# batra-mlp-lab/visdial

Hardware: AMD Instinct MI355X
Metric: QA-rounds/sec training mn-att-ques-im-hist+disc (batch 20x10x100) (higher is better)
Workload: dtype f32 operands and results; the option recurrence multiplies the EXACT 3-way bf16 split of both operands (9 bf16 MFMA products per fp32 product, f32 accumulate: fp32-grade, errors at the f32 MFMA's own level) -- its two step kernels and its weight-gradient contraction; f32 MFMA (v_mfma_f32_32x32x2_f32

## Files before the change

### visdial_amd/csrc/rt_core.h

```cpp
#pragma once
#include <math.h>
#include <stdarg.h>
#include <stdlib.h>
#include <string.h>

#include <algorithm>
#include <map>
#include <memory>
#include <numeric>
#include <random>
#include <string>
#include <vector>

#include "../../include/visdial_hip.h"
#include "common.h"
#include "paths.h"

int vd_lstm2_forward_p(const vd_lstm2_fwd_t* st, int nstacks, int H, int flags, hipStream_t stream);
int vd_lstm2_backward_p(const vd_lstm2_bwd_t* st, int nstacks, int H, int flags, hipStream_t stream);

int vd_img_drop_gather(const float* pre, const uint8_t* mask1, float* xdrop, int N, int R, int S2, int H, float scale, hipStream_t stream);
int vd_img_common_forward_p(const float* pre, const uint8_t* mask1, const float* xdrop, const float* Wc, const float* bc, const float* qc,
                            const uint8_t* mask2, float* iqc, int N, int R, int S2, int H, int Kc, float scale, int flags, hipStream_t stream);
int vd_img_tr_backward_p(const float* dz, const float* Wc, const float* p, const float* datt, const uint8_t* mask1, float* dpre, int N, int R,
// ... 123 lines not shown
  void flush() {
    index.reset(index.T);
    ++stamp;
  }
};
static constexpr long VD_OPTION_CACHE_DEFAULT_ROWS = 262144;
static constexpr long VD_OPTION_CACHE_FIRST_ROWS = 16384;

struct Encoder;
struct Decoder;

}

struct vd_model {
  vd_model_params p;
  int flags = 0;
  std::string enc_name, dec_name;
  std::vector<vdrt::Tensor> spec;
  std::map<std::string, int> index;
  long numel = 0;
  float *W = nullptr, *G = nullptr, *M = nullptr, *V = nullptr;
  std::map<std::string, vdrt::DevBuf> ws;
  std::map<std::string, vdrt::DevBuf> ext_masks;
  hipStream_t s_main = nullptr, s_enc = nullptr, s_img = nullptr, s_hist = nullptr, s_tab = nullptr, s_copy = nullptr;
  hipStream_t s_wg = nullptr;
  bool wg_active = false, wg_used = false;
  std::vector<hipEvent_t> ev_pool;
  size_t ev_next = 0;
  hipEvent_t ev_enc_grads = nullptr;
  hipEvent_t ev_updated = nullptr;
  bool updated_recorded = false;
  bool enc_grads_recorded = false;
  hipEvent_t ev_loss = nullptr, ev_prof[6] = {nullptr, nullptr, nullptr, nullptr, nullptr, nullptr};
  bool training = true, streams = true, prof_valid = false;
  long step = 0;
  int adam_t = 0;
  double lr = 1e-3;
  vdrt::BatchSlot slot[2];
  int cur = -1, uploaded = -1;
  float* loss_host = nullptr;
  long loss_cap = 0, loss_n = 0;
  bool loss_is_sum = false;
  std::unique_ptr<vdrt::Encoder> enc;
  std::unique_ptr<vdrt::Decoder> dec;
  float* scores = nullptr;
  float* gen_enc_out = nullptr;
  int gen_seq_len = 0;
// ... 42 lines not shown
}

inline void add_lstm(vd_model* m, const std::string& name, long D, long H) {
  m->spec.push_back(Tensor{name + ".W", 0, D + H, 4 * H, 1});
  m->spec.push_back(Tensor{name + ".b", 0, 1, 4 * H, 2});
}
inline void add_linear(vd_model* m, const std::string& name, long in, long out) {
  m->spec.push_back(Tensor{name + ".W", 0, out, in, 3});
  m->spec.push_back(Tensor{name + ".b", 0, 1, out, 4});
}
inline std::string hop_sfx(int i) { return i == 0 ? std::string() : std::to_string(i + 1); }

inline float* Wp(vd_model* m, const std::string& n) { return m->W + m->spec[m->index.at(n)].off; }
inline float* Gp(vd_model* m, const std::string& n) { return m->G + m->spec[m->index.at(n)].off; }

inline int fork_stream(vd_model* m, hipStream_t from, hipStream_t side) {
  if (side == from) return VD_OK;
  hipEvent_t e = m->ev_pool[m->ev_next++ % m->ev_pool.size()];
  VD_HIP(hipEventRecord(e, from));
  VD_HIP(hipStreamWaitEvent(side, e, 0));
  return VD_OK;
}
inline int join_stream(vd_model* m, hipStream_t side, hipStream_t to) { return fork_stream(m, side, to); }
inline hipStream_t side_stream(vd_model* m, hipStream_t wanted, hipStream_t cur) { return m->streams ? wanted : cur; }
inline int wg_fork(vd_model* m, hipStream_t cur, hipStream_t* out) {
  *out = cur;
  if (!m->wg_active || !m->s_wg) return VD_OK;
  VD_TRY(fork_stream(m, cur, m->s_wg));
  m->wg_used = true;
  *out = m->s_wg;
  return VD_OK;
}

inline int drop_mask(vd_model* m, const std::string& site, size_t numel, float p, hipStream_t s, uint8_t** out) {
  *out = nullptr;
  if (!m->training || p <= 0.f) return VD_OK;
  auto it = m->ext_masks.find(site);
  if (it != m->ext_masks.end()) {
    VD_CHECK_ARG(it->second.bytes >= numel, "dropout mask '%s' holds %zu bytes, the batch needs %zu", site.c_str(),
                 it->second.bytes, numel);
    *out = static_cast<uint8_t*>(it->second.p);
    return VD_OK;
  }
  if (!m->ext_masks.empty()) {
    vd_set_error("external dropout masks are set but none for site '%s'", site.c_str());
    return VD_ERR_STATE;
  }
// ... 300 lines not shown
```

### visdial_amd/csrc/rt_decoders.h

```cpp
#pragma once
#include "rt_encoders.h"

namespace vdrt {

int option_cache_resolve(vd_model* m, BatchSlot& sl, const int32_t* options, long NO, int To, hipStream_t s);

struct Decoder {
  virtual ~Decoder() {}
  virtual void declare(vd_model* m) = 0;
  virtual int forward_backward(vd_model* m, BatchSlot& b, bool only_forward) = 0;
  virtual int retrieve(vd_model* m, BatchSlot& b) = 0;
  virtual int retrieve_lhood(vd_model*, BatchSlot&) {
    vd_set_error("vd_model_retrieve_lhood: the live-row log-likelihood head scores candidates of decoder 'gen'; this model's decoder is 'disc'");
    return VD_ERR_ARG;
  }
  virtual int gen_begin(vd_model*, const int32_t*, int) { return no_gen(); }
  virtual int gen_step(vd_model*, const int32_t*, float*) { return no_gen(); }
  virtual int gen_select(vd_model*, const int32_t*, int) { return no_gen(); }
  virtual int gen_beam_search(vd_model*, int, int, int, int, int32_t*, double*) { return no_gen(); }
  virtual int gen_sample(vd_model*, int, int, int, double, const double*, int32_t*, double*) { return no_gen(); }
  static int no_gen() {
    vd_set_error("sampling / beam search only for the generative decoder (model.lua:436-438)");
    return VD_ERR_STATE;
  }
// ... 15 lines not shown

#ifdef VD_PROBE_PHASES
inline hipEvent_t* probe_events() {
  static hipEvent_t e[6];
  static bool made = false;
  if (!made) { for (auto& x : e) (void)hipEventCreate(&x); made = true; }
  return e;
}
#define VD_PROBE_REC(i, stream) (void)hipEventRecord(probe_events()[i], stream)
#else
#define VD_PROBE_REC(i, stream)
#endif
struct Disc : Decoder {
  void declare(vd_model* m) override { add_lstm(m, "opt", m->p.embedSize, m->p.rnnHiddenSize); }
  int forward_backward(vd_model* m, BatchSlot& b, bool only_forward) override {
    VD_CHECK_ARG(b.opt.present, "decoder 'disc' needs batch.options");
    VD_CHECK_ARG(only_forward || b.has_gt, "training decoder 'disc' needs batch.answer_ind");
    if (b.cached) return forward_cached(m, b, only_forward);
    const int N = b.q.N, O = m->p.numOptions, NOfull = N * O, NO = b.opt.N, To = b.opt.T;
    const bool dedup = b.opt_uid != nullptr;
    VD_CHECK_ARG(dedup ? NO <= NOfull : NO == NOfull, "decoder 'disc': %d option rows for %d x %d candidates", NO, N, O);
    const long H = m->p.rnnHiddenSize, E = m->p.embedSize, V = m->p.vocabSize;
    hipStream_t s = m->s_main;
    hipStream_t se = side_stream(m, m->s_enc, s);
    hipStream_t st = side_stream(m, m->s_tab, s);
    float *table, *gates, *h, *c, *scores, *loss_rows;
    VD_TRY(ws_get(m, "opt.table", (size_t)(V + 1) * 4 * H, &table));
    VD_TRY(ws_get(m, "opt.gates", (size_t)To * NO * 4 * H, &gates));
    VD_TRY(ws_get(m, "opt.h", (size_t)To * NO * H, &h));
    VD_TRY(ws_get(m, "opt.c", (size_t)To * NO * H, &c));
    VD_TRY(ws_get(m, "opt.scores", (size_t)N * O, &scores));
    VD_TRY(ws_get(m, "crit.loss_rows", (size_t)N, &loss_rows));
    float* Wopt = Wp(m, "opt.W");
    const int flags = m->flags;
    VD_TRY(fork_stream(m, s, se));
    float* enc_out = nullptr;
    VD_TRY(vd_gemm_nn(Wp(m, "embed"), E, Wopt, 4 * H, Wp(m, "opt.b"), table, 4 * H, (int)V + 1, (int)(4 * H), (int)E, 0, s));
    const bool c16 = (flags & VD_FLAG_BF16) && vd_lstm_c16_fits(NO, (int)H);
    vd_bf16_bits *gates16 = reinterpret_cast<vd_bf16_bits*>(gates), *h16 = reinterpret_cast<vd_bf16_bits*>(h), *table16 = nullptr;
    float* h_last = nullptr;
    if (c16) {
      float* t16;
      VD_TRY(ws_get(m, "opt.table16", (size_t)(V + 1) * 2 * H, &t16));
      VD_TRY(ws_get(m, "opt.h_last", (size_t)NO * H, &h_last));
      table16 = reinterpret_cast<vd_bf16_bits*>(t16);
      VD_TRY(vd_f32_to_bf16(table, table16, (V + 1) * 4 * H, s));
    }
    VD_HIP(hipEventRecord(m->ev_prof[0], s));
    {
      VdRange r("disc: option LSTM forward");
      if (c16) VD_TRY(vd_lstm_forward_c16(table16, 4 * H, b.opt.tok, Wopt + E * 4 * H, gates16, h16, h_last, c, To, NO, (int)H, s));
      else VD_TRY(vd_lstm_forward(table, 0, 4 * H, b.opt.tok, nullptr, Wopt + E * 4 * H, nullptr, nullptr, gates, h, c, To, NO, (int)H, flags, s));
    }
    VD_HIP(hipEventRecord(m->ev_prof[1], s));
    {
      VdRange r("encoder forward");
      VD_TRY(m->enc->forward(m, se, b, &enc_out));
      VD_PROBE_REC(0, se);
    }
    VD_TRY(join_stream(m, se, s));
    const float* optH = c16 ? h_last : h + (long)(To - 1) * NO * H;
    float *d_optH = nullptr, *d_enc = nullptr, *d_optH_full = nullptr;
    if (dedup) {
      float* full;
      VD_TRY(ws_get(m, "opt.h_full", (size_t)NOfull * H, &full));
      VD_TRY(vd_embed_gather(optH, b.opt_uid, nullptr, full, NOfull, (int)H, 1.f, s));
      optH = full;
    }
    if (!only_forward) {
      VD_TRY(ws_get(m, "crit.d_optH", (size_t)NO * H, &d_optH));
      VD_TRY(ws_get(m, "crit.d_enc", (size_t)N * H, &d_enc));
      if (dedup) VD_TRY(ws_get(m, "crit.d_optH_full", (size_t)NOfull * H, &d_optH_full));
    }
    VD_TRY(vd_score_ce(optH, enc_out, b.gt, scores, loss_rows, dedup ? d_optH_full : d_optH, d_enc, N, O, (int)H, 1.0f / N, s));
    if (dedup && !only_forward) {
      VD_TRY(vd_memset(d_optH, 0, (long)NO * H * 4, s));
      VD_TRY(vd_embed_scatter_acc(d_optH, b.opt_uid, nullptr, d_optH_full, NOfull, (int)H, 1.f, s));
    }
    VD_TRY(stage_loss(m, loss_rows, N, false, s));
    m->scores = scores;
    m->prof_valid = !only_forward;
    if (only_forward) return VD_OK;
    VD_TRY(fork_stream(m, s, se));
    float *dc, *dtab;
    int32_t* perm = b.opt_sort_perm;
    VD_TRY(ws_get(m, "opt.dc", (size_t)NO * H, &dc));
    VD_TRY(ws_get(m, "opt.dtable", (size_t)(V + 1) * 4 * H, &dtab));
    VD_CHECK_ARG(perm, "decoder 'disc': the batch slot carries no option-token sort");
    VD_TRY(fork_stream(m, s, st));
    VD_TRY(vd_memset(dtab, 0, (V + 1) * 4 * H * 4, st));
    VD_HIP(hipEventRecord(m->ev_prof[2], s));
    m->wg_active = m->streams && m->s_wg && (flags & VD_FLAG_BF16) != 0;
    m->wg_used = false;
    auto enc_bwd = [&]() -> int {
      VdRange r("encoder backward");
      VD_TRY(m->enc->backward(m, se, b, d_enc));
      VD_PROBE_REC(1, se);
      if (m->wg_used) VD_PROBE_REC(2, m->s_wg);
      if (m->wg_used) {
        VD_TRY(fork_stream(m, se, m->s_wg));
        VD_HIP(hipEventRecord(m->ev_enc_grads, m->s_wg));
      } else {
        VD_HIP(hipEventRecord(m->ev_enc_grads, se));
      }
      m->enc_grads_recorded = true;
      return VD_OK;
    };
    {
      VdRange r("disc: option LSTM backward");
      if (c16) VD_TRY(vd_lstm_backward_c16(Wopt + E * 4 * H, gates16, c, d_optH, dc, To, NO, (int)H, s));
      else VD_TRY(vd_lstm_backward(Wopt + E * 4 * H, gates, c, nullptr, nullptr, d_optH, nullptr, dc, nullptr, nullptr, nullptr, To, NO, (int)H, flags, s));
    }
    VD_HIP(hipEventRecord(m->ev_prof[3], s));
    VD_TRY(enc_bwd());
    VdRange rwg("disc: table gradient + dWh");
    VD_TRY(fork_stream(m, s, st));
    if (c16) VD_TRY(vd_segment_rowsum_acc_bf16(gates16, 4 * H, b.opt.tok, perm, (long)To * NO, (int)(4 * H), dtab, 4 * H, st));
    else VD_TRY(vd_segment_rowsum_acc(gates, 4 * H, b.opt.tok, perm, (long)To * NO, (int)(4 * H), dtab, 4 * H, st));
    VD_TRY(vd_colsum_acc(dtab, 4 * H, (int)V + 1, (int)(4 * H), Gp(m, "opt.b"), st));
    VD_TRY(vd_gemm_tn_acc(Wp(m, "embed"), E, dtab, 4 * H, Gp(m, "opt.W"), 4 * H, (int)E, (int)(4 * H), (int)V + 1, 0, st));
    VD_HIP(hipEventRecord(m->ev_prof[4], s));
    if (To > 1 && c16)
      VD_TRY(vd_gemm_tn_acc_bf16(h16, gates16 + (long)NO * 4 * H, Gp(m, "opt.W") + E * 4 * H, 4 * H, (int)H, (int)(4 * H), (To - 1) * NO, s));
    else if (To > 1)
      VD_TRY(vd_gemm_tn_acc(h, H, gates + (long)NO * 4 * H, 4 * H, Gp(m, "opt.W") + E * 4 * H, 4 * H, (int)H, (int)(4 * H), (To - 1) * NO,
                            flags & (VD_FLAG_BF16 | VD_FLAG_SPLIT9), s));
    VD_HIP(hipEventRecord(m->ev_prof[5], s));
    VD_TRY(vd_gemm_nt(dtab, 4 * H, Wopt, 4 * H, nullptr, Gp(m, "embed"), E, (int)V + 1, (int)E, (int)(4 * H), VD_ACT_NONE, 2, st));
    VD_PROBE_REC(3, st);
    VD_TRY(join_stream(m, se, s));
    if (m->wg_used) VD_TRY(join_stream(m, m->s_wg, s));
    m->wg_active = m->wg_used = false;
    VD_TRY(join_stream(m, st, s));
    VD_PROBE_REC(4, s);
    return VD_OK;
  }
  int retrieve(vd_model* m, BatchSlot& b) override { return forward_backward(m, b, true); }

  int forward_cached(vd_model* m, BatchSlot& b, bool only_forward) {
    if (!only_forward || m->training) {
      vd_set_error("decoder 'disc': this batch was uploaded for cached evaluation (VD_OPTION_CACHE with training off) and carries only the "
                   "candidate rows the cache did not hold; upload it again after vd_model_set_training(1) for a training step");
      return VD_ERR_STATE;
    }
    OptionCache& oc = m->ocache;
    const int N = b.q.N, O = m->p.numOptions, NOfull = N * O, To = b.opt.T;
    const long H = m->p.rnnHiddenSize, E = m->p.embedSize, V = m->p.vocabSize;
    hipStream_t s = m->s_main;
    hipStream_t se = side_stream(m, m->s_enc, s);
    if (b.cache_stamp != oc.stamp) {
      VD_HIP(hipEventSynchronize(b.ready));
      VD_TRY(option_cache_resolve(m, b, b.opt_host.data(), NOfull, To, s));
      VD_HIP(hipStreamSynchronize(s));
    }
    const int U = b.opt.N;
    const long count = oc.index.size();
    VD_CHECK_ARG(b.opt_total == NOfull && (long)b.miss_keys.size() == (long)U * To && count <= oc.capacity,
                 "decoder 'disc': inconsistent cached batch (%d candidates, %d misses)", b.opt_total, U);
    if (oc.table_rows < count + U) {
      const long want = std::min(std::max(2 * oc.table_rows, VD_OPTION_CACHE_FIRST_ROWS), oc.capacity);
      const long rows = std::max(want, count + U);
      float* nt = nullptr;
      VD_HIP(hipMalloc((void**)&nt, (size_t)rows * H * sizeof(float)));
      if (oc.table) {
        if (count > 0) VD_HIP(hipMemcpyAsync(nt, oc.table, (size_t)count * H * sizeof(float), hipMemcpyDeviceToDevice, s));
        VD_HIP(hipStreamSynchronize(s));
        VD_HIP(hipFree(oc.table));
      }
      oc.table = nt;
      oc.table_rows = rows;
    }
    float *scores, *loss_rows, *full;
    VD_TRY(ws_get(m, "opt.scores", (size_t)N * O, &scores));
    VD_TRY(ws_get(m, "crit.loss_rows", (size_t)N, &loss_rows));
    VD_TRY(ws_get(m, "opt.h_full", (size_t)NOfull * H, &full));
    VD_TRY(fork_stream(m, s, se));
    if (U > 0) {
      VdRange r("disc: option LSTM forward (state only, cache misses)");
      float *table, *h, *c;
      VD_TRY(ws_get(m, "opt.table", (size_t)(V + 1) * 4 * H, &table));
      VD_TRY(ws_get(m, "opt.h2", (size_t)2 * U * H, &h));
      VD_TRY(ws_get(m, "opt.c2", (size_t)2 * U * H, &c));
      float* Wopt = Wp(m, "opt.W");
      VD_TRY(vd_gemm_nn(Wp(m, "embed"), E, Wopt, 4 * H, Wp(m, "opt.b"), table, 4 * H, (int)V + 1, (int)(4 * H), (int)E, 0, s));
      VD_TRY(vd_lstm_forward(table, 0, 4 * H, b.opt.tok, nullptr, Wopt + E * 4 * H, nullptr, nullptr, nullptr, h, c, To, U, (int)H,
                             m->flags | VD_FLAG_STATE_ONLY, s));
      VD_HIP(hipMemcpyAsync(oc.table + count * H, h + (long)((To - 1) & 1) * U * H, (size_t)U * H * sizeof(float), hipMemcpyDeviceToDevice, s));
      const long fit = std::min<long>(U, oc.capacity - count);
      for (long i = 0; i < fit; ++i) oc.index.add(b.miss_keys.data() + (size_t)i * To);
    }
    ++oc.stamp;
    float* enc_out = nullptr;
    {
      VdRange r("encoder forward");
      VD_TRY(m->enc->forward(m, se, b, &enc_out));
    }
    VD_TRY(join_stream(m, se, s));
    VD_TRY(vd_embed_gather(oc.table, b.opt_uid, nullptr, full, NOfull, (int)H, 1.f, s));
    VD_TRY(vd_score_ce(full, enc_out, b.gt, scores, loss_rows, nullptr, nullptr, N, O, (int)H, 1.0f / N, s));
    VD_TRY(stage_loss(m, loss_rows, N, false, s));
    m->scores = scores;
    m->prof_valid = false;
    return VD_OK;
  }
};

struct Gen;
int Gen_begin(Gen* g, vd_model* m, const int32_t* rounds, int n);
int Gen_step(Gen* g, vd_model* m, const int32_t* tokens, float* host_logp);
int Gen_select(Gen* g, vd_model* m, const int32_t* src, int n_keep);
int Gen_beam_search(Gen* g, vd_model* m, int k, int L, int start, int end, int32_t* host_tokens, double* host_scores);
int Gen_sample(Gen* g, vd_model* m, int L, int start, int end, double T, const double* host_u, int32_t* host_tokens,
               double* host_loglik);

struct Gen : Decoder {
  int gen_begin(vd_model* m, const int32_t* r, int n) override { return Gen_begin(this, m, r, n); }
  int gen_step(vd_model* m, const int32_t* t, float* lp) override { return Gen_step(this, m, t, lp); }
  int gen_select(vd_model* m, const int32_t* src, int k) override { return Gen_select(this, m, src, k); }
  int gen_beam_search(vd_model* m, int k, int L, int st, int en, int32_t* t, double* sc) override {
    return Gen_beam_search(this, m, k, L, st, en, t, sc);
// ... 453 lines not shown
```

### visdial_amd/csrc/rt_encoders.h

```cpp
#pragma once
#include "rt_core.h"

namespace vdrt {

struct Encoder {
  virtual ~Encoder() {}
  virtual void declare(vd_model* m) = 0;
  virtual int forward(vd_model* m, hipStream_t s, BatchSlot& b, float** out) = 0;
  virtual int backward(vd_model* m, hipStream_t s, BatchSlot& b, const float* grad_out) = 0;
  virtual std::vector<SeqLSTM>* rnnLayers() { return nullptr; }
  virtual int seqLen(const BatchSlot& b) const { return b.q.T; }
};

inline int tick_flags(const vd_model* m) { return m->flags & VD_FLAG_BF16; }

inline int causal_mask(vd_model* m, int B, int R, uint8_t** out) {
  const std::string key = "causal." + std::to_string(B);
  DevBuf& d = m->ws[key];
  const size_t n = (size_t)B * R * R;
  if (!d.p) {
    std::vector<uint8_t> host(n);
    for (int r = 0; r < B * R; ++r)
      for (int j = 0; j < R; ++j) host[(size_t)r * R + j] = j > (r % R) ? 1 : 0;
    VD_HIP(hipMalloc(&d.p, n + 16));
// ... 224 lines not shown
  std::vector<float*> iqc, patt;
  float sc = 1.f;
  float* xdrop = nullptr;
  int iflags = 0;
  static void declare(vd_model* m) {
    const long H = m->p.rnnHiddenSize, C = m->p.imgFeatureSize, K = m->p.commonEmbeddingSize;
    add_linear(m, "img_proj", C, H);
    for (int i = 0; i < std::max(1, m->p.numAttentionLayers); ++i) {
      add_linear(m, "img_common" + hop_sfx(i), H, K);
      add_linear(m, "ques_common" + hop_sfx(i), H, K);
      add_linear(m, "att" + hop_sfx(i), K, 1);
    }
    add_linear(m, "out", H, H);
  }
  void init(vd_model* m) {
    H = m->p.rnnHiddenSize; C = m->p.imgFeatureSize; K = m->p.commonEmbeddingSize;
    S2 = m->p.imgSpatialSize * m->p.imgSpatialSize; R = m->p.maxQuesCount; L = std::max(1, m->p.numAttentionLayers);
    img_proj.init("img_proj", C, H); out.init("out", H, H);
    ques_common.resize(L);
    for (int i = 0; i < L; ++i) ques_common[i].init("ques_common" + hop_sfx(i), H, K);
  }
  int prefetch(vd_model* m, hipStream_t s, BatchSlot& b, int N_) {
    N = N_;
    hipStream_t si = side_stream(m, m->s_img, s);
    VD_TRY(fork_stream(m, s, si));
    VD_TRY(img_proj.forward(m, si, b.img, (long)b.B * S2, true, &pre));
    VD_TRY(drop_mask(m, "img_tr", (size_t)N * S2 * H, 0.5f, si, &m1));
    m2.assign(L, nullptr);
    for (int i = 0; i < L; ++i) VD_TRY(drop_mask(m, "iqc" + hop_sfx(i), (size_t)N * S2 * K, 0.5f, si, &m2[i]));
    sc = m1 ? 2.f : 1.f;
    iflags = (m->flags & VD_FLAG_SPLIT9) && vd_img_split_ok((long)N * S2, (int)H, (int)K) ? VD_FLAG_SPLIT9 : 0;
    xdrop = nullptr;
    if (iflags) {
      VD_TRY(ws_get(m, "att.xdrop", (size_t)N * S2 * H, &xdrop));
      VD_TRY(vd_img_drop_gather(pre, m1, xdrop, N, R, S2, (int)H, sc, si));
    }
    return VD_OK;
  }
  int forward(vd_model* m, hipStream_t s, const float* u0, float** y) {
    VD_TRY(join_stream(m, side_stream(m, m->s_img, s), s));
    u_in.assign(L, nullptr); iqc.assign(L, nullptr); patt.assign(L, nullptr);
    const float* u = u0;
    for (int i = 0; i < L; ++i) {
      const std::string sf = hop_sfx(i);
      float *qc, *u1;
      VD_TRY(ques_common[i].forward(m, s, u, N, false, &qc));
      VD_TRY(ws_get(m, "att.iqc" + sf, (size_t)N * S2 * K, &iqc[i]));
      VD_TRY(ws_get(m, "att.p" + sf, (size_t)N * S2, &patt[i]));
      VD_TRY(ws_get(m, "att.u1" + sf, (size_t)N * H, &u1));
      VD_TRY(vd_img_common_forward_p(pre, m1, xdrop, Wp(m, "img_common" + sf + ".W"), Wp(m, "img_common" + sf + ".b"), qc, m2[i], iqc[i], N, R,
                                     S2, (int)H, (int)K, sc, iflags, s));
      VD_TRY(vd_img_att_forward(iqc[i], Wp(m, "att" + sf + ".W"), Wp(m, "att" + sf + ".b"), pre, m1, u, patt[i], u1, N, R, S2, (int)H,
                                (int)K, sc, s));
      u_in[i] = u;
      u = u1;
    }
    VD_TRY(drop_mask(m, "u", (size_t)N * H, 0.5f, s, &m_u));
    const float* ud;
    VD_TRY(dropout_fwd(m, "att.u1_d", u, m_u, 2.f, (long)N * H, s, &ud));
    return out.forward(m, s, ud, N, true, y);
  }
  int backward(vd_model* m, hipStream_t s, BatchSlot& b, const float* grad_out, float** du0) {
    float* du1d;
// ... 120 lines not shown
    rnn.resize(L);
    for (int l = 0; l < L; ++l) {
      add_lstm(m, "ques" + std::to_string(l + 1), l == 0 ? E : H, H);
      rnn[l].init("ques" + std::to_string(l + 1), l == 0 ? E : H, H);
    }
    if (use_hist) {
      hist.resize(L);
      for (int l = 0; l < L; ++l) {
        add_lstm(m, "hist" + std::to_string(l + 1), l == 0 ? E : H, H);
        hist[l].init("hist" + std::to_string(l + 1), l == 0 ? E : H, H);
      }
    }
    std::vector<long> dims = {H};
    if (use_im) dims.push_back(F);
    if (use_hist) dims.push_back(H);
    long D = 0;
    for (long d : dims) D += d;
    add_linear(m, "fuse", D, H);
    fuse.init("fuse", dims, H);
  }
  std::vector<SeqLSTM>* rnnLayers() override { return &rnn; }
  int forward(vd_model* m, hipStream_t s, BatchSlot& b, float** out) override {
    const int N = b.q.N, Tq = b.q.T, R = m->p.maxQuesCount;
    hipStream_t sh = side_stream(m, m->s_hist, s);
    const float* hh_last = nullptr;
    if (use_hist) {
      VD_TRY(fork_stream(m, s, sh));
      const int Th = b.h.T;
      const bool prof = m->dec_name == "gen";
      if (prof) VD_HIP(hipEventRecord(m->ev_prof[0], sh));
      if (HistWave::usable(b, hist)) {
        VD_TRY(wave.forward(m, sh, b, hist[0], hist[1], &hh_last));
      } else {
        float *hx, *ht;
        VD_TRY(ws_get(m, "h.x", (size_t)Th * N * E, &hx));
        VD_TRY(vd_embed_gather(Wp(m, "embed"), b.h.tok, nullptr, hx, (long)Th * N, (int)E, 1.f, sh));
        VD_TRY(lstm_stack_forward(m, sh, hist, {hx}, Th, N, b.h.tok, &ht));
        hh_last = hist.back().out_at(Th - 1);
      }
      if (prof) VD_HIP(hipEventRecord(m->ev_prof[1], sh));
    }
    float *qx, *qt;
    VD_TRY(ws_get(m, "q.x", (size_t)Tq * N * E, &qx));
    VD_TRY(vd_embed_gather(Wp(m, "embed"), b.q.tok, nullptr, qx, (long)Tq * N, (int)E, 1.f, s));
    VD_TRY(lstm_stack_forward(m, s, rnn, {qx}, Tq, N, b.q.tok, &qt));
    std::vector<const float*> parts = {rnn.back().out_at(Tq - 1)};
    if (use_im) {
      int32_t* rep;
      float* img_rep;
      VD_TRY(round_index(m, N, R, &rep));
      VD_TRY(ws_get(m, "img.rep", (size_t)N * F, &img_rep));
      VD_TRY(vd_embed_gather(b.img, rep, nullptr, img_rep, N, (int)F, 1.f, s));
      parts.push_back(img_rep);
    }
    if (use_hist) {
      VD_TRY(join_stream(m, sh, s));
      parts.push_back(hh_last);
    }
    uint8_t* mk;
    VD_TRY(drop_mask(m, "fuse", (size_t)N * fuse.D, pdrop, s, &mk));
    return fuse.forward(m, s, parts, N, mk, pdrop > 0.f ? 1.f / (1.f - pdrop) : 1.f, out);
  }
  int backward(vd_model* m, hipStream_t s, BatchSlot& b, const float* grad_out) override {
    std::vector<bool> need = {true};
    if (use_im) need.push_back(false);
    if (use_hist) need.push_back(true);
    std::vector<float*> g;
    VD_TRY(fuse.backward(m, s, grad_out, need, &g));
    hipStream_t sh = side_stream(m, m->s_hist, s);
    if (use_hist) {
      VD_TRY(fork_stream(m, s, sh));
      const bool prof = m->dec_name == "gen";
      if (prof) VD_HIP(hipEventRecord(m->ev_prof[2], sh));
      if (HistWave::usable(b, hist)) {
        VD_TRY(wave.backward(m, sh, b, hist[0], hist[1], g.back()));
      } else {
        std::vector<float*> dx;
        VD_TRY(lstm_stack_backward(m, sh, hist, g.back(), nullptr, &dx));
        VD_TRY(vd_embed_scatter_acc(Gp(m, "embed"), b.h.tok, nullptr, dx[0], (long)b.h.T * b.h.N, (int)E, 1.f, sh));
      }
      if (prof) VD_HIP(hipEventRecord(m->ev_prof[3], sh));
      m->prof_hist = prof;
    }
    std::vector<float*> dx;
    VD_TRY(lstm_stack_backward(m, s, rnn, g[0], nullptr, &dx));
    VD_TRY(vd_embed_scatter_acc(Gp(m, "embed"), b.q.tok, nullptr, dx[0], (long)b.q.T * b.q.N, (int)E, 1.f, s));
    if (use_hist) VD_TRY(join_stream(m, sh, s));
    return VD_OK;
  }
};

struct Hre : Encoder {
// ... 27 lines not shown
    if (attention) {
      add_linear(m, "att_q", H, 1);
      add_linear(m, "att_h", H, 1);
    }
    add_lstm(m, "dialog", 2 * H, H);
    dialog.init("dialog", 2 * H, H, {H, H});
  }
  std::vector<SeqLSTM>* rnnLayers() override { return &rnn; }
  int indices(vd_model* m, int N, int32_t** rep, int32_t** to_rb, int32_t** to_n) {
    const int B = N / R;
    std::vector<int32_t> a(N), c(N);
    for (int n = 0; n < N; ++n) {
      a[n] = (n % B) * R + n / B;
      c[n] = (n % R) * B + n / R;
    }
    VD_TRY(round_index(m, N, R, rep));
    VD_TRY(index_array(m, "idx.to_rb." + std::to_string(N), a, to_rb));
    return index_array(m, "idx.to_n." + std::to_string(N), c, to_n);
  }
  int forward(vd_model* m, hipStream_t s, BatchSlot& b, float** out) override {
    const int N = b.q.N, Tq = b.q.T, Th = b.h.T, B = N / R;
    int32_t *rep, *to_rb, *to_n;
    VD_TRY(indices(m, N, &rep, &to_rb, &to_n));
    hipStream_t sh = side_stream(m, m->s_hist, s);
    VD_TRY(fork_stream(m, s, sh));
    if (HistWave::usable(b, hist)) {
      const float* last;
      VD_TRY(wave.forward(m, sh, b, hist[0], hist[1], &last));
      hh = const_cast<float*>(last);
    } else {
      float *hx, *ht;
      VD_TRY(ws_get(m, "h.x", (size_t)Th * N * E, &hx));
      VD_TRY(vd_embed_gather(Wp(m, "embed"), b.h.tok, nullptr, hx, (long)Th * N, (int)E, 1.f, sh));
      VD_TRY(lstm_stack_forward(m, sh, hist, {hx}, Th, N, b.h.tok, &ht));
      hh = hist.back().out_at(Th - 1);
    }
    float* qx;
    VD_TRY(ws_get(m, "q.x", (size_t)Tq * N * E, &qx));
    VD_TRY(vd_embed_gather(Wp(m, "embed"), b.q.tok, nullptr, qx, (long)Tq * N, (int)E, 1.f, s));
    std::vector<const float*> x = {qx};
    if (use_im) {
      float *img_rep, *imgE, *xi;
      VD_TRY(ws_get(m, "img.rep", (size_t)N * F, &img_rep));
      VD_TRY(vd_embed_gather(b.img, rep, nullptr, img_rep, N, (int)F, 1.f, s));
      m_img = nullptr;
      if (attention) VD_TRY(drop_mask(m, "img", (size_t)N * F, 0.5f, s, &m_img));
      const float* img_in;
// ... 42 lines not shown
    VD_TRY(vd_embed_gather(grad_out, to_rb, nullptr, g_rb, N, (int)H, 1.f, s));
    std::vector<float*> dd;
    VD_TRY(dialog.backward(m, s, g_rb, nullptr, {}, &dd));
    VD_TRY(vd_embed_gather(dd[0], to_n, nullptr, dfirst, N, (int)H, 1.f, s));
    VD_TRY(vd_embed_gather(dd[1], to_n, nullptr, dsecond, N, (int)H, 1.f, s));
    const float *dq = dfirst, *dh = dsecond;
    if (attention) {
      float *dsq, *dsh, *dh_att, *dq_s, *dh_s, *dqq, *dhh;
      VD_TRY(ws_get(m, "hrea.dsq", (size_t)N, &dsq));
      VD_TRY(ws_get(m, "hrea.dsh", (size_t)N, &dsh));
      VD_TRY(ws_get(m, "hrea.dh", (size_t)N * H, &dh_att));
      VD_TRY(ws_get(m, "hrea.dq_s", (size_t)N * H, &dq_s));
      VD_TRY(ws_get(m, "hrea.dh_s", (size_t)N * H, &dh_s));
      VD_TRY(ws_get(m, "hrea.dq", (size_t)N * H, &dqq));
      VD_TRY(ws_get(m, "hrea.dhh", (size_t)N * H, &dhh));
      VD_TRY(vd_hrea_attention_backward(hh, P, dfirst, dsq, dsh, dh_att, B, R, (int)H, s));
      VD_TRY(vd_rowdot_backward(hq, Wp(m, "att_q.W"), dsq, Gp(m, "att_q.W"), Gp(m, "att_q.b"), dq_s, N, (int)H, s));
      VD_TRY(vd_rowdot_backward(hh, Wp(m, "att_h.W"), dsh, Gp(m, "att_h.W"), Gp(m, "att_h.b"), dh_s, N, (int)H, s));
      VD_TRY(vd_axpby(dsecond, dq_s, dqq, (long)N * H, 1.f, 1.f, s));
      VD_TRY(vd_axpby(dh_att, dh_s, dhh, (long)N * H, 1.f, 1.f, s));
      dq = dqq;
      dh = dhh;
    }
    hipStream_t sh = side_stream(m, m->s_hist, s);
    VD_TRY(fork_stream(m, s, sh));
    if (HistWave::usable(b, hist)) {
      VD_TRY(wave.backward(m, sh, b, hist[0], hist[1], dh));
    } else {
      std::vector<float*> dx;
      VD_TRY(lstm_stack_backward(m, sh, hist, dh, nullptr, &dx));
      VD_TRY(vd_embed_scatter_acc(Gp(m, "embed"), b.h.tok, nullptr, dx[0], (long)b.h.T * N, (int)E, 1.f, sh));
    }
    std::vector<float*> dx;
    VD_TRY(lstm_stack_backward(m, s, rnn, dq, nullptr, &dx));
    VD_TRY(vd_embed_scatter_acc(Gp(m, "embed"), b.q.tok, nullptr, dx[0], (long)Tq * N, (int)E, 1.f, s));
    if (use_im) {
      float* dimgE;
      VD_TRY(ws_get(m, "q.dimgE", (size_t)N * DI, &dimgE));
      VD_TRY(vd_mask_time_backward(dx[1], b.q.tok, dimgE, Tq, N, (int)DI, s));
      VD_TRY(img_embed.backward(m, s, dimgE, false, nullptr));
    }
    return join_stream(m, sh, s);
  }
};

inline std::unique_ptr<Encoder> make_encoder(const std::string& n) {
  if (n == "mn-att-ques-im-hist" || n == "mn-ques-hist" || n == "mn-ques-im-hist" || n == "lf-att-ques-im-hist")
// ... 13 lines not shown
```

### visdial_amd/csrc/runtime.hip

```cpp
#include "rt_decoders.h"

using namespace vdrt;

vd_model::~vd_model() {}

namespace {

int upload_tokens(BatchSlot& sl, SeqTok& ss, const std::string& tag, const int32_t* rows_major, int N, int T, bool sorted, hipStream_t s) {
  ss.T = T;
  ss.N = N;
  ss.present = true;
  ss.sorted = sorted;
  const size_t TN = (size_t)T * N;
  const size_t total = sorted ? 7 * TN + 2 * (size_t)N + T : TN;
  int32_t* stage = nullptr;
  VD_TRY(pin_get(sl.pinned, tag + ".stage", total * sizeof(int32_t), (void**)&stage));
  int32_t* tok = stage;
  std::vector<int> len(sorted ? N : 0);
  for (int n = 0; n < N; ++n) {
    int first = T;
    for (int t = 0; t < T; ++t) {
      const int32_t v = rows_major[(size_t)n * T + t];
      tok[(size_t)t * N + n] = v;
      if (v != 0 && first == T) first = t;
// ... 278 lines not shown
  m->enc->declare(m);
  m->dec->declare(m);
  long off = 0;
  for (size_t i = 0; i < m->spec.size(); ++i) {
    m->spec[i].off = off;
    m->index[m->spec[i].name] = (int)i;
    off += (m->spec[i].numel() + 3) / 4 * 4;
  }
  m->numel = off;
  auto fail = [&](int rc) {
    vd_model_destroy(m);
    return rc;
  };
  for (float** v : {&m->W, &m->G, &m->M, &m->V}) {
    if (hipMalloc((void**)v, off * sizeof(float)) != hipSuccess) {
      vd_set_error("vd_model_create: hipMalloc of %ld floats failed", off);
      return fail(VD_ERR_HIP);
    }
    (void)hipMemset(*v, 0, off * sizeof(float));
  }
  int least = 0, greatest = 0;
  (void)hipDeviceGetStreamPriorityRange(&least, &greatest);
  if (hipStreamCreateWithPriority(&m->s_main, hipStreamNonBlocking, least) != hipSuccess) return fail(VD_ERR_HIP);
  for (hipStream_t* s : {&m->s_enc, &m->s_img, &m->s_copy})
    if (hipStreamCreateWithPriority(s, hipStreamNonBlocking, greatest) != hipSuccess) return fail(VD_ERR_HIP);
  const int tab_prio = greatest;
  if (hipStreamCreateWithPriority(&m->s_tab, hipStreamNonBlocking, tab_prio) != hipSuccess) return fail(VD_ERR_HIP);
  if (least - greatest >= 2 &&
      hipStreamCreateWithPriority(&m->s_wg, hipStreamNonBlocking, (least + greatest) / 2) != hipSuccess)
    return fail(VD_ERR_HIP);
  m->s_hist = m->s_img;
  m->ev_pool.resize(64);
  for (auto& e : m->ev_pool)
    if (hipEventCreateWithFlags(&e, hipEventDisableTiming) != hipSuccess) return fail(VD_ERR_HIP);
  if (hipEventCreateWithFlags(&m->ev_loss, hipEventDisableTiming) != hipSuccess) return fail(VD_ERR_HIP);
  if (hipEventCreateWithFlags(&m->ev_enc_grads, hipEventDisableTiming) != hipSuccess) return fail(VD_ERR_HIP);
  if (hipEventCreateWithFlags(&m->ev_updated, hipEventDisableTiming) != hipSuccess) return fail(VD_ERR_HIP);
  for (auto& e : m->ev_prof)
    if (hipEventCreate(&e) != hipSuccess) return fail(VD_ERR_HIP);
  for (auto& sl : m->slot)
    if (hipEventCreateWithFlags(&sl.ready, hipEventDisableTiming) != hipSuccess ||
        hipEventCreateWithFlags(&sl.done, hipEventDisableTiming) != hipSuccess)
      return fail(VD_ERR_HIP);
  *out = m;
  return VD_OK;
}

void vd_model_destroy(vd_model* m) {
  if (!m) return;
  (void)hipDeviceSynchronize();
  for (float* v : {m->W, m->G, m->M, m->V})
    if (v) (void)hipFree(v);
  for (auto& kv : m->ws)
    if (kv.second.p) (void)hipFree(kv.second.p);
  for (auto& kv : m->ext_masks)
    if (kv.second.p) (void)hipFree(kv.second.p);
  if (m->ocache.table) (void)hipFree(m->ocache.table);
  for (auto& sl : m->slot) {
    for (auto& kv : sl.bufs)
      if (kv.second.p) (void)hipFree(kv.second.p);
    for (auto& kv : sl.pinned)
      if (kv.second.p) (void)hipHostFree(kv.second.p);
    if (sl.ready) (void)hipEventDestroy(sl.ready);
    if (sl.done) (void)hipEventDestroy(sl.done);
  }
  if (m->loss_host) (void)hipHostFree(m->loss_host);
  for (auto& e : m->ev_pool)
    if (e) (void)hipEventDestroy(e);
  if (m->ev_loss) (void)hipEventDestroy(m->ev_loss);
  if (m->ev_enc_grads) (void)hipEventDestroy(m->ev_enc_grads);
  if (m->ev_updated) (void)hipEventDestroy(m->ev_updated);
  for (auto& e : m->ev_prof)
    if (e) (void)hipEventDestroy(e);
  for (hipStream_t s : {m->s_main, m->s_enc, m->s_img, m->s_tab, m->s_copy, m->s_wg})
    if (s) {
      (void)hipStreamDestroy(s);
    }
  delete m;
}

int64_t vd_model_num_tensors(const vd_model* m) { return m ? (int64_t)m->spec.size() : 0; }
int64_t vd_model_flat_size(const vd_model* m) { return m ? m->numel : 0; }

int vd_model_tensor_info(const vd_model* m, int64_t i, char* name64, int64_t* offset, int64_t* rows, int64_t* cols) {
  VD_CHECK_ARG(m && i >= 0 && i < (int64_t)m->spec.size(), "vd_model_tensor_info: bad index");
  const Tensor& t = m->spec[i];
  if (name64) {
    strncpy(name64, t.name.c_str(), 63);
    name64[63] = 0;
  }
  if (offset) *offset = t.off;
  if (rows) *rows = t.rows;
  if (cols) *cols = t.cols;
  return VD_OK;
}

int vd_model_flat_pointers(vd_model* m, float** W, float** dW, float** adam_m, float** adam_v) {
// ... 80 lines not shown
  VD_CHECK_ARG(m, "vd_model_set_dropout_mask: null model");
  VD_HIP(hipStreamSynchronize(m->s_main));
  if (!host) {
    for (auto& kv : m->ext_masks)
      if (kv.second.p) VD_HIP(hipFree(kv.second.p));
    m->ext_masks.clear();
    return VD_OK;
  }
  VD_CHECK_ARG(site && n > 0, "vd_model_set_dropout_mask: bad arguments");
  void* p = nullptr;
  VD_TRY(dev_get(m->ext_masks, site, (size_t)n, &p));
  VD_HIP(hipMemcpy(p, host, (size_t)n, hipMemcpyHostToDevice));
  return VD_OK;
}

int vd_model_upload_batch(vd_model* m, const vd_batch* hb) {
  VD_CHECK_ARG(m && hb && hb->ques_fwd && hb->B > 0 && hb->Tq > 0, "vd_model_upload_batch: missing ques_fwd / B / Tq");
  VD_CHECK_ARG(!m->use_hist || (hb->hist && hb->Th > 0), "vd_model_upload_batch: encoder '%s' needs hist", m->enc_name.c_str());
  VD_CHECK_ARG(!m->use_im || hb->img_feat, "vd_model_upload_batch: encoder '%s' needs img_feat", m->enc_name.c_str());
  const bool disc = m->dec_name == "disc";
  VD_CHECK_ARG(!disc || (hb->options && hb->To > 0), "vd_model_upload_batch: decoder 'disc' needs options");
  VdRange r("vd_model_upload_batch");
  BatchSlot& sl = m->slot[m->cur < 0 ? 0 : (m->cur ^ 1)];
  hipStream_t s = m->s_copy;
  if (sl.used) VD_HIP(hipStreamWaitEvent(s, sl.done, 0));
  if (sl.uploaded) VD_HIP(hipEventSynchronize(sl.ready));
  sl.uploaded = true;
  sl.B = hb->B;
  const int R = m->p.maxQuesCount, N = hb->B * R, O = m->p.numOptions;
  const long NO = (long)N * O;
  for (SeqTok* t : {&sl.q, &sl.h, &sl.opt, &sl.ain, &sl.aout, &sl.oin, &sl.oout}) t->present = false;
  VD_TRY(upload_tokens(sl, sl.q, "q", hb->ques_fwd, N, hb->Tq, m->is_graph, s));
  const bool hist_wave = !m->is_graph && m->p.numLayers == 2;
  if (m->use_hist) VD_TRY(upload_tokens(sl, sl.h, "h", hb->hist, N, hb->Th, m->is_graph || hist_wave, s));
  if (m->use_im) {
    const size_t img_n = (size_t)hb->B * (m->is_att ? (size_t)m->p.imgSpatialSize * m->p.imgSpatialSize : 1) * m->p.imgFeatureSize;
    float* ip = nullptr;
    VD_TRY(pin_get(sl.pinned, "img.stage", img_n * sizeof(float), (void**)&ip));
    memcpy(ip, hb->img_feat, img_n * sizeof(float));
    VD_TRY(dev_get(sl.bufs, "img", img_n * sizeof(float), (void**)&sl.img));
    VD_HIP(hipMemcpyAsync(sl.img, ip, img_n * sizeof(float), hipMemcpyHostToDevice, s));
  }
  if (disc) {
    sl.opt_uid = nullptr;
    sl.opt_total = (int)NO;
    sl.cached = false;
    const int To = hb->To;
// ... 229 lines not shown
    for (int i = 1; i < 6; ++i) (void)hipEventElapsedTime(&t[i], m->ev_prof[0], m->ev_prof[i]);
    for (int i = 0; i < 5; ++i) (void)hipEventElapsedTime(&t[6 + i], m->ev_prof[0], pe[i]);
    fprintf(stderr, "PHASES (ms after option-fwd start) main: fwd end %.2f | bwd %.2f -> %.2f | dWh %.2f -> %.2f | all joined %.2f  ||  enc fwd end %.2f | enc bwd chain end %.2f | "
            "wg chain end %.2f | table chain end %.2f\n", t[1], t[2], t[3], t[4], t[5], t[10], t[6], t[7], t[8], t[9]); }
#endif
  return VD_OK;
}

int vd_model_option_rows(vd_model* m, int64_t* executed, int64_t* total) {
  VD_CHECK_ARG(m && executed && total && (m->cur >= 0 || m->uploaded >= 0), "vd_model_option_rows: no batch uploaded");
  if (m->lhood_exec >= 0) {
    *executed = m->lhood_exec;
    *total = m->lhood_total;
    return VD_OK;
  }
  const BatchSlot& b = m->slot[m->cur >= 0 ? m->cur : m->uploaded];
  *executed = b.opt.present ? b.opt.N : 0;
  *total = b.opt.present ? (b.opt_total ? b.opt_total : b.opt.N) : 0;
  return VD_OK;
}

int vd_model_synchronize(vd_model* m) {
  VD_CHECK_ARG(m, "vd_model_synchronize: null model");
  for (hipStream_t s : {m->s_copy, m->s_enc, m->s_img, m->s_tab, m->s_wg, m->s_main})
    if (s) VD_HIP(hipStreamSynchronize(s));
  return VD_OK;
}

}
```

Baseline: 8265.

## Collapse encoder, image, history, table and copy streams into one side stream

Replaces the separate encoder, image, history, table-gradient and upload-copy streams with a single high-priority side stream. All work that used to fork onto those streams now serialises on one side queue alongside the main stream. This cuts the number of streams and the cross-stream event waits, but gives up concurrency that existed before: the batch upload, image prefetch, encoder, and table-gradient work can no longer overlap with each other.

```diff
diff --git a/visdial_amd/csrc/rt_core.h b/visdial_amd/csrc/rt_core.h
--- a/visdial_amd/csrc/rt_core.h
+++ b/visdial_amd/csrc/rt_core.h
@@ -169,7 +169,7 @@
   float *W = nullptr, *G = nullptr, *M = nullptr, *V = nullptr;
   std::map<std::string, vdrt::DevBuf> ws;
   std::map<std::string, vdrt::DevBuf> ext_masks;
-  hipStream_t s_main = nullptr, s_enc = nullptr, s_img = nullptr, s_hist = nullptr, s_tab = nullptr, s_copy = nullptr;
+  hipStream_t s_main = nullptr, s_side = nullptr;
   hipStream_t s_wg = nullptr;
   bool wg_active = false, wg_used = false;
   std::vector<hipEvent_t> ev_pool;
@@ -258,7 +258,7 @@
   return VD_OK;
 }
 inline int join_stream(vd_model* m, hipStream_t side, hipStream_t to) { return fork_stream(m, side, to); }
-inline hipStream_t side_stream(vd_model* m, hipStream_t wanted, hipStream_t cur) { return m->streams ? wanted : cur; }
+inline hipStream_t side_stream(vd_model* m, hipStream_t cur) { return m->streams ? m->s_side : cur; }
 inline int wg_fork(vd_model* m, hipStream_t cur, hipStream_t* out) {
   *out = cur;
   if (!m->wg_active || !m->s_wg) return VD_OK;
diff --git a/visdial_amd/csrc/rt_decoders.h b/visdial_amd/csrc/rt_decoders.h
--- a/visdial_amd/csrc/rt_decoders.h
+++ b/visdial_amd/csrc/rt_decoders.h
@@ -61,8 +61,7 @@
     VD_CHECK_ARG(dedup ? NO <= NOfull : NO == NOfull, "decoder 'disc': %d option rows for %d x %d candidates", NO, N, O);
     const long H = m->p.rnnHiddenSize, E = m->p.embedSize, V = m->p.vocabSize;
     hipStream_t s = m->s_main;
-    hipStream_t se = side_stream(m, m->s_enc, s);
-    hipStream_t st = side_stream(m, m->s_tab, s);
+    hipStream_t sd = side_stream(m, s);
     float *table, *gates, *h, *c, *scores, *loss_rows;
     VD_TRY(ws_get(m, "opt.table", (size_t)(V + 1) * 4 * H, &table));
     VD_TRY(ws_get(m, "opt.gates", (size_t)To * NO * 4 * H, &gates));
@@ -72,7 +71,7 @@
     VD_TRY(ws_get(m, "crit.loss_rows", (size_t)N, &loss_rows));
     float* Wopt = Wp(m, "opt.W");
     const int flags = m->flags;
-    VD_TRY(fork_stream(m, s, se));
+    VD_TRY(fork_stream(m, s, sd));
     float* enc_out = nullptr;
     VD_TRY(vd_gemm_nn(Wp(m, "embed"), E, Wopt, 4 * H, Wp(m, "opt.b"), table, 4 * H, (int)V + 1, (int)(4 * H), (int)E, 0, s));
     const bool c16 = (flags & VD_FLAG_BF16) && vd_lstm_c16_fits(NO, (int)H);
@@ -94,10 +93,10 @@
     VD_HIP(hipEventRecord(m->ev_prof[1], s));
     {
       VdRange r("encoder forward");
-      VD_TRY(m->enc->forward(m, se, b, &enc_out));
-      VD_PROBE_REC(0, se);
-    }
-    VD_TRY(join_stream(m, se, s));
+      VD_TRY(m->enc->forward(m, sd, b, &enc_out));
+      VD_PROBE_REC(0, sd);
+    }
+    VD_TRY(join_stream(m, sd, s));
     const float* optH = c16 ? h_last : h + (long)(To - 1) * NO * H;
     float *d_optH = nullptr, *d_enc = nullptr, *d_optH_full = nullptr;
     if (dedup) {
@@ -120,27 +119,26 @@
     m->scores = scores;
     m->prof_valid = !only_forward;
     if (only_forward) return VD_OK;
-    VD_TRY(fork_stream(m, s, se));
+    VD_TRY(fork_stream(m, s, sd));
     float *dc, *dtab;
     int32_t* perm = b.opt_sort_perm;
     VD_TRY(ws_get(m, "opt.dc", (size_t)NO * H, &dc));
     VD_TRY(ws_get(m, "opt.dtable", (size_t)(V + 1) * 4 * H, &dtab));
     VD_CHECK_ARG(perm, "decoder 'disc': the batch slot carries no option-token sort");
-    VD_TRY(fork_stream(m, s, st));
-    VD_TRY(vd_memset(dtab, 0, (V + 1) * 4 * H * 4, st));
+    VD_TRY(vd_memset(dtab, 0, (V + 1) * 4 * H * 4, sd));
     VD_HIP(hipEventRecord(m->ev_prof[2], s));
     m->wg_active = m->streams && m->s_wg && (flags & VD_FLAG_BF16) != 0;
     m->wg_used = false;
     auto enc_bwd = [&]() -> int {
       VdRange r("encoder backward");
-      VD_TRY(m->enc->backward(m, se, b, d_enc));
-      VD_PROBE_REC(1, se);
+      VD_TRY(m->enc->backward(m, sd, b, d_enc));
+      VD_PROBE_REC(1, sd);
       if (m->wg_used) VD_PROBE_REC(2, m->s_wg);
       if (m->wg_used) {
-        VD_TRY(fork_stream(m, se, m->s_wg));
+        VD_TRY(fork_stream(m, sd, m->s_wg));
         VD_HIP(hipEventRecord(m->ev_enc_grads, m->s_wg));
       } else {
-        VD_HIP(hipEventRecord(m->ev_enc_grads, se));
+        VD_HIP(hipEventRecord(m->ev_enc_grads, sd));
       }
       m->enc_grads_recorded = true;
       return VD_OK;
@@ -153,11 +151,11 @@
     VD_HIP(hipEventRecord(m->ev_prof[3], s));
     VD_TRY(enc_bwd());
     VdRange rwg("disc: table gradient + dWh");
-    VD_TRY(fork_stream(m, s, st));
-    if (c16) VD_TRY(vd_segment_rowsum_acc_bf16(gates16, 4 * H, b.opt.tok, perm, (long)To * NO, (int)(4 * H), dtab, 4 * H, st));
-    else VD_TRY(vd_segment_rowsum_acc(gates, 4 * H, b.opt.tok, perm, (long)To * NO, (int)(4 * H), dtab, 4 * H, st));
-    VD_TRY(vd_colsum_acc(dtab, 4 * H, (int)V + 1, (int)(4 * H), Gp(m, "opt.b"), st));
-    VD_TRY(vd_gemm_tn_acc(Wp(m, "embed"), E, dtab, 4 * H, Gp(m, "opt.W"), 4 * H, (int)E, (int)(4 * H), (int)V + 1, 0, st));
+    VD_TRY(fork_stream(m, s, sd));
+    if (c16) VD_TRY(vd_segment_rowsum_acc_bf16(gates16, 4 * H, b.opt.tok, perm, (long)To * NO, (int)(4 * H), dtab, 4 * H, sd));
+    else VD_TRY(vd_segment_rowsum_acc(gates, 4 * H, b.opt.tok, perm, (long)To * NO, (int)(4 * H), dtab, 4 * H, sd));
+    VD_TRY(vd_colsum_acc(dtab, 4 * H, (int)V + 1, (int)(4 * H), Gp(m, "opt.b"), sd));
+    VD_TRY(vd_gemm_tn_acc(Wp(m, "embed"), E, dtab, 4 * H, Gp(m, "opt.W"), 4 * H, (int)E, (int)(4 * H), (int)V + 1, 0, sd));
     VD_HIP(hipEventRecord(m->ev_prof[4], s));
     if (To > 1 && c16)
       VD_TRY(vd_gemm_tn_acc_bf16(h16, gates16 + (long)NO * 4 * H, Gp(m, "opt.W") + E * 4 * H, 4 * H, (int)H, (int)(4 * H), (To - 1) * NO, s));
@@ -165,12 +163,11 @@
       VD_TRY(vd_gemm_tn_acc(h, H, gates + (long)NO * 4 * H, 4 * H, Gp(m, "opt.W") + E * 4 * H, 4 * H, (int)H, (int)(4 * H), (To - 1) * NO,
                             flags & (VD_FLAG_BF16 | VD_FLAG_SPLIT9), s));
     VD_HIP(hipEventRecord(m->ev_prof[5], s));
-    VD_TRY(vd_gemm_nt(dtab, 4 * H, Wopt, 4 * H, nullptr, Gp(m, "embed"), E, (int)V + 1, (int)E, (int)(4 * H), VD_ACT_NONE, 2, st));
-    VD_PROBE_REC(3, st);
-    VD_TRY(join_stream(m, se, s));
+    VD_TRY(vd_gemm_nt(dtab, 4 * H, Wopt, 4 * H, nullptr, Gp(m, "embed"), E, (int)V + 1, (int)E, (int)(4 * H), VD_ACT_NONE, 2, sd));
+    VD_PROBE_REC(3, sd);
+    VD_TRY(join_stream(m, sd, s));
     if (m->wg_used) VD_TRY(join_stream(m, m->s_wg, s));
     m->wg_active = m->wg_used = false;
-    VD_TRY(join_stream(m, st, s));
     VD_PROBE_REC(4, s);
     return VD_OK;
   }
@@ -186,7 +183,7 @@
     const int N = b.q.N, O = m->p.numOptions, NOfull = N * O, To = b.opt.T;
     const long H = m->p.rnnHiddenSize, E = m->p.embedSize, V = m->p.vocabSize;
     hipStream_t s = m->s_main;
-    hipStream_t se = side_stream(m, m->s_enc, s);
+    hipStream_t sd = side_stream(m, s);
     if (b.cache_stamp != oc.stamp) {
       VD_HIP(hipEventSynchronize(b.ready));
       VD_TRY(option_cache_resolve(m, b, b.opt_host.data(), NOfull, To, s));
@@ -213,7 +210,7 @@
     VD_TRY(ws_get(m, "opt.scores", (size_t)N * O, &scores));
     VD_TRY(ws_get(m, "crit.loss_rows", (size_t)N, &loss_rows));
     VD_TRY(ws_get(m, "opt.h_full", (size_t)NOfull * H, &full));
-    VD_TRY(fork_stream(m, s, se));
+    VD_TRY(fork_stream(m, s, sd));
     if (U > 0) {
       VdRange r("disc: option LSTM forward (state only, cache misses)");
       float *table, *h, *c;
@@ -232,9 +229,9 @@
     float* enc_out = nullptr;
     {
       VdRange r("encoder forward");
-      VD_TRY(m->enc->forward(m, se, b, &enc_out));
-    }
-    VD_TRY(join_stream(m, se, s));
+      VD_TRY(m->enc->forward(m, sd, b, &enc_out));
+    }
+    VD_TRY(join_stream(m, sd, s));
     VD_TRY(vd_embed_gather(oc.table, b.opt_uid, nullptr, full, NOfull, (int)H, 1.f, s));
     VD_TRY(vd_score_ce(full, enc_out, b.gt, scores, loss_rows, nullptr, nullptr, N, O, (int)H, 1.0f / N, s));
     VD_TRY(stage_loss(m, loss_rows, N, false, s));
diff --git a/visdial_amd/csrc/rt_encoders.h b/visdial_amd/csrc/rt_encoders.h
--- a/visdial_amd/csrc/rt_encoders.h
+++ b/visdial_amd/csrc/rt_encoders.h
@@ -270,7 +270,7 @@
   }
   int prefetch(vd_model* m, hipStream_t s, BatchSlot& b, int N_) {
     N = N_;
-    hipStream_t si = side_stream(m, m->s_img, s);
+    hipStream_t si = side_stream(m, s);
     VD_TRY(fork_stream(m, s, si));
     VD_TRY(img_proj.forward(m, si, b.img, (long)b.B * S2, true, &pre));
     VD_TRY(drop_mask(m, "img_tr", (size_t)N * S2 * H, 0.5f, si, &m1));
@@ -286,7 +286,7 @@
     return VD_OK;
   }
   int forward(vd_model* m, hipStream_t s, const float* u0, float** y) {
-    VD_TRY(join_stream(m, side_stream(m, m->s_img, s), s));
+    VD_TRY(join_stream(m, side_stream(m, s), s));
     u_in.assign(L, nullptr); iqc.assign(L, nullptr); patt.assign(L, nullptr);
     const float* u = u0;
     for (int i = 0; i < L; ++i) {
@@ -453,7 +453,7 @@
   std::vector<SeqLSTM>* rnnLayers() override { return &rnn; }
   int forward(vd_model* m, hipStream_t s, BatchSlot& b, float** out) override {
     const int N = b.q.N, Tq = b.q.T, R = m->p.maxQuesCount;
-    hipStream_t sh = side_stream(m, m->s_hist, s);
+    hipStream_t sh = side_stream(m, s);
     const float* hh_last = nullptr;
     if (use_hist) {
       VD_TRY(fork_stream(m, s, sh));
@@ -498,7 +498,7 @@
     if (use_hist) need.push_back(true);
     std::vector<float*> g;
     VD_TRY(fuse.backward(m, s, grad_out, need, &g));
-    hipStream_t sh = side_stream(m, m->s_hist, s);
+    hipStream_t sh = side_stream(m, s);
     if (use_hist) {
       VD_TRY(fork_stream(m, s, sh));
       const bool prof = m->dec_name == "gen";
@@ -572,7 +572,7 @@
     const int N = b.q.N, Tq = b.q.T, Th = b.h.T, B = N / R;
     int32_t *rep, *to_rb, *to_n;
     VD_TRY(indices(m, N, &rep, &to_rb, &to_n));
-    hipStream_t sh = side_stream(m, m->s_hist, s);
+    hipStream_t sh = side_stream(m, s);
     VD_TRY(fork_stream(m, s, sh));
     if (HistWave::usable(b, hist)) {
       const float* last;
@@ -661,7 +661,7 @@
       dq = dqq;
       dh = dhh;
     }
-    hipStream_t sh = side_stream(m, m->s_hist, s);
+    hipStream_t sh = side_stream(m, s);
     VD_TRY(fork_stream(m, s, sh));
     if (HistWave::usable(b, hist)) {
       VD_TRY(wave.backward(m, sh, b, hist[0], hist[1], dh));
diff --git a/visdial_amd/csrc/runtime.hip b/visdial_amd/csrc/runtime.hip
--- a/visdial_amd/csrc/runtime.hip
+++ b/visdial_amd/csrc/runtime.hip
@@ -324,14 +324,10 @@
   int least = 0, greatest = 0;
   (void)hipDeviceGetStreamPriorityRange(&least, &greatest);
   if (hipStreamCreateWithPriority(&m->s_main, hipStreamNonBlocking, least) != hipSuccess) return fail(VD_ERR_HIP);
-  for (hipStream_t* s : {&m->s_enc, &m->s_img, &m->s_copy})
-    if (hipStreamCreateWithPriority(s, hipStreamNonBlocking, greatest) != hipSuccess) return fail(VD_ERR_HIP);
-  const int tab_prio = greatest;
-  if (hipStreamCreateWithPriority(&m->s_tab, hipStreamNonBlocking, tab_prio) != hipSuccess) return fail(VD_ERR_HIP);
+  if (hipStreamCreateWithPriority(&m->s_side, hipStreamNonBlocking, greatest) != hipSuccess) return fail(VD_ERR_HIP);
   if (least - greatest >= 2 &&
       hipStreamCreateWithPriority(&m->s_wg, hipStreamNonBlocking, (least + greatest) / 2) != hipSuccess)
     return fail(VD_ERR_HIP);
-  m->s_hist = m->s_img;
   m->ev_pool.resize(64);
   for (auto& e : m->ev_pool)
     if (hipEventCreateWithFlags(&e, hipEventDisableTiming) != hipSuccess) return fail(VD_ERR_HIP);
@@ -374,7 +370,7 @@
   if (m->ev_updated) (void)hipEventDestroy(m->ev_updated);
   for (auto& e : m->ev_prof)
     if (e) (void)hipEventDestroy(e);
-  for (hipStream_t s : {m->s_main, m->s_enc, m->s_img, m->s_tab, m->s_copy, m->s_wg})
+  for (hipStream_t s : {m->s_main, m->s_side, m->s_wg})
     if (s) {
       (void)hipStreamDestroy(s);
     }
@@ -501,7 +497,7 @@
   VD_CHECK_ARG(!disc || (hb->options && hb->To > 0), "vd_model_upload_batch: decoder 'disc' needs options");
   VdRange r("vd_model_upload_batch");
   BatchSlot& sl = m->slot[m->cur < 0 ? 0 : (m->cur ^ 1)];
-  hipStream_t s = m->s_copy;
+  hipStream_t s = m->s_side;
   if (sl.used) VD_HIP(hipStreamWaitEvent(s, sl.done, 0));
   if (sl.uploaded) VD_HIP(hipEventSynchronize(sl.ready));
   sl.uploaded = true;
@@ -777,7 +773,7 @@
 
 int vd_model_synchronize(vd_model* m) {
   VD_CHECK_ARG(m, "vd_model_synchronize: null model");
-  for (hipStream_t s : {m->s_copy, m->s_enc, m->s_img, m->s_tab, m->s_wg, m->s_main})
+  for (hipStream_t s : {m->s_side, m->s_wg, m->s_main})
     if (s) VD_HIP(hipStreamSynchronize(s));
   return VD_OK;
 }
```

After: 9002, median of 6. 8.9% higher.
